# Makiato1999/HRI-EMO

Measured on AMD Instinct MI355X. Metric: utterances/sec fwd+bwd, d=768 T_a=400 T_t=128 N_e=6, higher is better.
Workload: dtype bf16; 1 GPU; FusionWithEmotionDecoder fwd+bwd (train mode, dropout 0.1), d=768 T_a=400 T_t=128 N_e=6 H=8, 2 fusion + 2 decoder layers, all-False masks (BASELINE cfg2); global_batch=64, batch_per_gpu=64, parallelism=dp1, grad_allreduce=none, launch=hipGraph replay, streams=2

## Files before the change

### hri-emo_amd/_lib.py

```python
import ctypes
import os

_HERE = os.path.dirname(os.path.abspath(__file__))
LIB_PATH = os.environ.get("HRIEMO_LIB") or os.path.join(_HERE, "libhriemo.so")

_C = {"p": ctypes.c_void_p, "i": ctypes.c_int, "l": ctypes.c_long, "f": ctypes.c_float,
      "Q": ctypes.c_ulonglong, "I": ctypes.c_uint}

_SIGS = {
    "hriemo_gemm_bf16": ("iiiiiplplplipipliplp", "i"),
    "hriemo_gemm_force_config": ("i", "i"),
    "hriemo_gemm_debug_flags": ("i", "i"),
    "hriemo_gemm_colsum_rows": ("iiiii", "i"),
    "hriemo_gemm_plan": ("iiiiiilppp", "i"),
    "hriemo_gemm_bf16_group_tn": ("piip", "i"),
    "hriemo_gemm_bf16_split": ("iiiiiplplplpliiplp", "i"),
    "hriemo_gemm_bf16_colsum": ("iiiiiplplplplpp", "i"),
    "hriemo_mx8_scale_ld": ("i", "l"),
    "hriemo_quant_mx8": ("pliiiplplp", "i"),
    "hriemo_gemm_mx8": ("iiiplplplplplipiplp", "i"),
    "hriemo_gemm_mx8_q": ("iiiplplplplplpiplplp", "i"),
    "hriemo_gemm_mx8_force_config": ("i", "i"),
    "hriemo_attn_fwd": ("plplplplppiiiiifQpIipp", "i"),
    "hriemo_attn_fwd_q": ("plplplplppiiiiifQpIipplplp", "i"),
    "hriemo_attn_bwd": ("plplplplplplplplpppiiiiifQpIipppp", "i"),
    "hriemo_attn_fwd_varlen": ("plplplplpppiiiiifQpIipp", "i"),
    "hriemo_attn_fwd_q_varlen": ("plplplplpppiiiiifQpIipplpllp", "i"),
    "hriemo_attn_bwd_varlen": ("plplplplplplplplppppiiiiifQpIipppp", "i"),
    "hriemo_attn_mask_bytes": ("iiii", "l"),
    "hriemo_attn_bwd_single_pass": ("iiii", "i"),
    "hriemo_attn_bwd_single_pass_q": ("iiiii", "i"),
    "hriemo_attn_bwd_kv_colsum_rows": ("iiiii", "i"),
    "hriemo_attn_bwd_colsum_rows": ("iiii", "i"),
    "hriemo_attn_bwd_dq_colsum_rows": ("iiiii", "i"),
    "hriemo_attn_plan": ("iiiiiipppppp", "i"),
    "hriemo_split_bf16x3": ("pliipiip", "i"),
    "hriemo_attn_fwd_f32": ("plplplplppiiiiifQpIip", "i"),
    "hriemo_attn_probs_f32": ("plplpppiiiiifQpIip", "i"),
# ... 122 lines not shown
```

### hri-emo_amd/_ops.py

```python
import itertools
import os as _os
import threading
from collections import namedtuple

import torch

from . import _lib

BF16 = torch.bfloat16
_EPS = 1e-5
_apply_tls = threading.local()


def _stream():
    return torch.cuda.current_stream().cuda_stream


def _p(t):
    return None if t is None else t.data_ptr()


def _require_fp32_master(p):
    if p.dtype != torch.float32:
        raise TypeError(f"hri_emo_amd: parameter of dtype {p.dtype}; keep the module's parameters in fp32 "
# ... 440 lines not shown

def fold_ffn_bias():
    return FOLD_FFN_BIAS


def linear_dx_masked_colsum(dy, w16, aux, bias_out, accumulate):
    M, N = dy.shape
    K = w16.shape[1]
    dx = torch.empty((M, K), dtype=BF16, device=dy.device)
    rows = _lib.lib().hriemo_gemm_colsum_rows(0, 1, M, K, N)
    part = torch.empty(rows * K, dtype=torch.float32, device=dy.device)
    _lib.call("hriemo_gemm_bf16_colsum", 0, 1, M, K, N, _p(dy), dy.stride(0), _p(w16), w16.stride(0), _p(dx), K, _p(aux), aux.stride(0),
              _p(part), _stream())
    if accumulate and DEFER_REDUCE and _in_backward():
        _deferred.add(part, K, rows, K, 1, [bias_out], True)
    else:
        red = _DeferredReduce()
        red.device = dy.device
        red.add(part, K, rows, K, 1, [bias_out], accumulate, schedule=False)
        red.flush()
    return dx


def linear_dw(dy, x, out, accumulate=False):
    M, N = dy.shape
    K = x.shape[1]
    if accumulate and M <= SMALL_DW_ROWS and _small_dw.enabled():
        _small_dw.add(dy, x, out)
        return
    gemm(1, 1, N, K, M, dy, dy.stride(0), x, x.stride(0), out, out.stride(0), c_f32=True, accumulate=accumulate)


def linear_dw_split(dy, x, out, out2, split, accumulate=False):
    M, N = dy.shape
    K = x.shape[1]
    ws = workspace(64 << 20, out.device)
    _lib.call("hriemo_gemm_bf16_split", 1, 1, N, K, M, _p(dy), dy.stride(0), _p(x), x.stride(0), _p(out), out.stride(0), _p(out2),
              out2.stride(0), split, int(accumulate), _p(ws), ws.numel() * 4, _stream())


GEMM_MODE = None


def set_gemm_mode(mode):
    global GEMM_MODE
    if mode not in ("bf16", "mx_fp8"):
        raise ValueError(f"gemm mode {mode!r}: expected 'bf16' or 'mx_fp8'")
    GEMM_MODE = mode


def gemm_mode():
    global GEMM_MODE
    if GEMM_MODE is None:
        import os
        GEMM_MODE = os.environ.get("HRIEMO_GEMM", "bf16")
        if GEMM_MODE not in ("bf16", "mx_fp8"):
            raise ValueError(f"HRIEMO_GEMM={GEMM_MODE!r}: expected 'bf16' or 'mx_fp8'")
    return GEMM_MODE


PRECISION = None
# ... 1001 lines not shown

def _attn_ln_fwd(ctx, head, q, k, v, x2, x32v, ar, H, hd, sh, w_in16, w_out16, drop, need_w, out_l, shape):
    p, seed, site, b_off = drop
    _, _, w_out, b_out, gamma, beta = ctx.params
    o, lse, *mbits = attn_fwd(q, k, v, ar.B, H, ar.Lq, ar.Lk, hd, ar.kpm, p, seed, site, b_off,
                              want_bits=attn_mask_bits(ar.B, H, ar.Lk, hd, ar.Lq), cu=ar.cu)
    g, y, y32, mean, rstd, mx = _proj_ln(o, sh, w_out, w_out16, b_out, x2, x32v, gamma, beta, p, seed, site + 1, b_off * ar.stride,
                                         ar.rows)
    probs = attn_probs(q, k, ar.B, H, ar.Lq, ar.Lk, hd, ar.kpm, lse, p, seed, site, b_off, ar.cu, out_l) if need_w else None
    ctx.save_for_backward(*head, o, lse, g, mean, rstd, w_in16, w_out16, gamma, mbits[0] if mbits else None)
    ctx.rows = ar
    ctx.mark_non_differentiable(*([probs] if probs is not None else []))
    return tag_mx(y.view(shape), mx), (y32.view(shape) if y32 is not None else None), probs


def _ln_bwd(params, dy, dy32, g, x2, x32v, gamma, mean, rstd, p, seed, site, row_off, rows, want_dx=True):
    dy2 = _contig_bf16(_sum_grads(dy, dy32)).view(x2.shape)
    sink = GradSink(params)
    return (sink,) + add_ln_bwd(dy2, g, x2, gamma, mean, rstd, p, seed, site, row_off, want_dx=want_dx,
                                outs=(sink.buf(params[-2]), sink.buf(params[-1]), sink.buf(params[-3])),
                                accumulate=sink.fused, x32=x32v, rows=rows)


def _attn_ln_bwd(ctx, params, dy, dy32, x2, x32v, tail, want_dx=True):
    o, lse, g, mean, rstd, w_in16, w_out16, gamma, mbits = tail
    p, seed, site, b_off = ctx.cfg[-4:]
    sink, ds, dg, dgamma, dbeta, db_out = _ln_bwd(params, dy, dy32, g, x2, x32v, gamma, mean, rstd, p, seed, site + 1,
                                                  b_off * ctx.rows.stride, ctx.rows.rows, want_dx)
    dw_out = sink.buf(params[-4])
    linear_dw(dg, o, dw_out, sink.fused)
    return sink, ds, linear_dx(dg, w_out16), dw_out, db_out, dgamma, dbeta


class SelfAttnLN(_GradModeAware, torch.autograd.Function):

    @staticmethod
    def forward(ctx, x, x32, w_in, b_in, w_out, b_out, gamma, beta, sh, H, seq, p, seed, site, b_off, need_w):
        seq.holds(x)
        if precision() == "fp32":
            return _fp32().self_attn_ln(ctx, x, x32, w_in, b_in, w_out, b_out, gamma, beta, sh, H, seq, need_w, p, seed, site, b_off)
        _require_fp32_masters(w_in, b_in, w_out, b_out, gamma, beta)
        ctx.set_materialize_grads(False)
        _require_gpu(x)
        B, L, d = x.shape
        hd = _heads(d, H)
        M = B * L
        ar = attn_rows(seq, seq, need_w)
        x2 = _contig_bf16(x).view(M, d)
        x32 = _c32(x32)
        x32v = x32.view(M, d) if x32 is not None else None
        w_in16, w_out16 = sh.get(w_in), sh.get(w_out)
        ctx.cfg = (B, L, d, H, hd, p, seed, site, b_off)
        ctx.params = (w_in, b_in, w_out, b_out, gamma, beta)
        qkv = proj_fwd(Operand(x2, mx_of(x)), sh, w_in, w_in16, b_in)
        return _attn_ln_fwd(ctx, (x2, x32v, qkv), qkv[:, :d], qkv[:, d:2 * d], qkv[:, 2 * d:], x2, x32v, ar, H, hd, sh, w_in16,
                            w_out16, (p, seed, site, b_off), need_w, (seq.L, seq.L), (B, L, d))

    @staticmethod
    def backward(ctx, dy, dy32, _dprobs):
        if getattr(ctx, "fp32", False):
            return _fp32().self_attn_ln_bwd(ctx, dy, dy32)
        x2, x32v, qkv, o, lse, _, _, _, w_in16, _, _, mbits = saved = ctx.saved_tensors
        B, L, d, H, hd, p, seed, site, b_off = ctx.cfg
        ar = ctx.rows
        M = B * L
        p_w_in, p_b_in = ctx.params[:2]
        want_dx = ctx.needs_input_grad[0] or ctx.needs_input_grad[1] or FORCE_INPUT_GRAD
        sink, ds, do, dw_out, db_out, dgamma, dbeta = _attn_ln_bwd(ctx, ctx.params, dy, dy32, x2, x32v, saved[-9:], want_dx)
        acc = sink.fused
        dqkv = torch.empty((M, 3 * d), dtype=BF16, device=x2.device)
        db_in = sink.buf(p_b_in)
        folded = attn_bwd(qkv[:, :d], qkv[:, d:2 * d], qkv[:, 2 * d:], o, do, dqkv[:, :d], dqkv[:, d:2 * d], dqkv[:, 2 * d:],
                          lse, ar.B, H, ar.Lq, ar.Lk, hd, ar.kpm, p, seed, site, b_off, bias_grad=(db_in[:d], db_in[d:], acc), mask_bits=mbits,
                          cu=ar.cu)
        dw_in = sink.buf(p_w_in)
        linear_dw(dqkv, x2, dw_in, acc)
        if not folded:
            colsum(dqkv, db_in, acc)
        dx = linear_dx(dqkv, w_in16, epi=3, aux=ds).view(B, L, d) if want_dx else None
        sink.done()
        if site in FLUSH_SITES:
            _small_dw.flush()
        r = sink.ret
        return (dx, None, r(dw_in), r(db_in), r(dw_out), r(db_out), r(dgamma), r(dbeta)) + (None,) * 8


class CrossAttnLN(_GradModeAware, torch.autograd.Function):

    @staticmethod
    def forward(ctx, xq, xq32, xkv, w_in, b_in, w_out, b_out, gamma, beta, sh, H, seq_q, seq_k, p, seed, site, b_off, need_w,
                kv_pre=None, join_q=None, q_pre=None, slots=None):
        if (q_pre is None) != (slots is None) or (q_pre is not None and kv_pre is None):
            raise ValueError("CrossAttnLN: q_pre and slots come together, and only with kv_pre (both projections made by SharedProjFn)")
        seq_q.holds(xq)
        seq_k.holds(xkv)
        if precision() == "fp32":
            return _fp32().cross_attn_ln(ctx, xq, xq32, xkv, w_in, b_in, w_out, b_out, gamma, beta, sh, H, seq_q, seq_k, need_w, p, seed,
                                         site, b_off)
        _require_fp32_masters(w_in, b_in, w_out, b_out, gamma, beta)
# ... 9 lines not shown
        ctx.cfg = (B, Lq, Lk, d, H, hd, p, seed, site, b_off)
        ctx.params = (w_in, b_in, w_out, b_out, gamma, beta)
        ctx.own_q, ctx.own_kv, ctx.slots, ctx.join_q = q_pre is None, kv_pre is None, slots, join_q
        w_out16 = sh.get(w_out)
        w_in16 = sh.get(w_in) if (ctx.own_q or ctx.own_kv) else None
        q = q_pre if q_pre is not None else proj_fwd(Operand(xq2, mx_of(xq)), sh, w_in, w_in16, b_in, rows=(0, d))
        if kv_pre is not None:
            xkv2, kv = None, kv_pre
        else:
            xkv2 = _contig_bf16(xkv).view(B * Lk, d)
            kv = proj_fwd(Operand(xkv2, mx_of(xkv)), sh, w_in, w_in16, b_in, rows=(d, 3 * d))
        return _attn_ln_fwd(ctx, (xq2, x32v, xkv2, q, kv), q, kv[:, :d], kv[:, d:], xq2, x32v, ar, H, hd, sh, w_in16,
                            w_out16, (p, seed, site, b_off), need_w, (seq_q.L, seq_k.L), (B, Lq, d))

    @staticmethod
    def backward(ctx, dy, dy32, _dprobs):
        if getattr(ctx, "fp32", False):
            return _fp32().cross_attn_ln_bwd(ctx, dy, dy32)
        xq2, x32v, xkv2, q, kv, o, lse, _, _, _, w_in16, _, _, mbits = saved = ctx.saved_tensors
        B, Lq, Lk, d, H, hd, p, seed, site, b_off = ctx.cfg
        ar = ctx.rows
        own_q, own_kv = ctx.own_q, ctx.own_kv
        p_w_in, p_b_in = ctx.params[:2]
        sink, ds, do, dw_out, db_out, dgamma, dbeta = _attn_ln_bwd(ctx, ctx.params if own_q else ctx.params[1:], dy, dy32, xq2, x32v, saved[-9:])
        acc = sink.fused
        if own_q:
            dq = torch.empty((B * Lq, d), dtype=BF16, device=xq2.device)
            dkv = (torch.zeros if ar.kv_surplus else torch.empty)((B * Lk, 2 * d), dtype=BF16, device=xq2.device)
        else:
            dq, dkv = ctx.slots[0].buf(), ctx.slots[1].buf()
        db_in = sink.buf(p_b_in)
        folded = attn_bwd(q, kv[:, :d], kv[:, d:], o, do, dq, dkv[:, :d], dkv[:, d:], lse, ar.B, H, ar.Lq, ar.Lk, hd, ar.kpm, p, seed,
                          site, b_off, bias_grad=(db_in[:d], db_in[d:], acc), mask_bits=mbits, cu=ar.cu)
        dw_in = None
        if own_q:
            dw_in = sink.buf(p_w_in)
            linear_dw(dq, xq2, dw_in[:d], acc)
        if not folded:
            colsum(dq, db_in[:d], acc)
            colsum(dkv, db_in[d:], acc)
        dxq = linear_dx(dq, w_in16[:d], epi=3, aux=ds) if own_q else ds
        if ctx.join_q is not None:
            last, dep = ctx.join_q.arrive()
            if dep is not None:
                dxq = dxq + dep.view(B * Lq, d)
            if not last:
                ctx.join_q.deposit(dxq)
                dxq = None
        dxq = dxq.view(B, Lq, d) if dxq is not None else None
        dxkv = None
        if own_kv:
            linear_dw(dkv, xkv2, dw_in[d:], acc)
            dxkv = linear_dx(dkv, w_in16[d:]).view(B, Lk, d)
        elif own_q and not acc:
            dw_in[d:].zero_()
        sink.done(skip=() if own_kv else (p_w_in,))
        r = sink.ret
        return (dxq, None, dxkv, r(dw_in), r(db_in), r(dw_out), r(db_out), r(dgamma), r(dbeta)) + (None,) * 9 + \
            (None if own_kv else dkv, None, None if own_q else dq, None)


class GradJoin:

    def __init__(self, n=2):
        self.n, self.seen, self.dep, self.ev = n, 0, None, None

    def arrive(self):
        if self.seen == 0:
            torch.autograd.Variable._execution_engine.queue_callback(self._check)
        self.seen += 1
        last = self.seen == self.n
        dep, ev = self.dep, self.ev
        self.dep = self.ev = None
        if last:
            self.seen = 0
# ... 204 lines not shown
                DROP_LOG.append(("rows", seed, site + 2, M, h.shape[1], float(p_mid), b_off * L))
            _lib.call("hriemo_dropout_bf16", _p(h), _p(hd_), M, h.shape[1], float(p_mid), seed, _p(seed_word(h.device)),
                      site + 2, b_off * L, _stream())
        g, y, y32, mean, rstd, mx = _proj_ln(hd_, sh, w2, w2_16, b2, x2, x32v, gamma, beta, p, seed, site + 1, b_off * seq.L, seq.idx)
        ctx.save_for_backward(x2, x32v, h, hd_, g, mean, rstd, w1_16, w2_16, gamma)
        ctx.cfg = (B, L, d, p, p_mid, seed, site, b_off)
        ctx.seq = seq
        ctx.params = (w1, b1, w2, b2, gamma, beta)
        return tag_mx(y.view(B, L, d), mx), (y32.view(B, L, d) if y32 is not None else None)

    @staticmethod
    def backward(ctx, dy, dy32):
        if getattr(ctx, "fp32", False):
            return _fp32().ffn_ln_bwd(ctx, dy, dy32)
        x2, x32v, h, hd_, g, mean, rstd, w1_16, w2_16, gamma = ctx.saved_tensors
        B, L, d, p, p_mid, seed, site, b_off = ctx.cfg
        M, F = h.shape
        dev = x2.device
        p_w1, p_b1, p_w2 = ctx.params[:3]
        sink, ds, dg, dgamma, dbeta, db2 = _ln_bwd(ctx.params, dy, dy32, g, x2, x32v, gamma, mean, rstd, p, seed, site + 1,
                                                   b_off * ctx.seq.L, ctx.seq.idx)
        acc = sink.fused
        dw2 = sink.buf(p_w2)
        linear_dw(dg, hd_, dw2, acc)
        db1 = sink.buf(p_b1)
        fold = p_mid == 0 and fold_ffn_bias()
        if fold:
            da = linear_dx_masked_colsum(dg, w2_16, h, db1, acc)
        else:
            da = linear_dx(dg, w2_16, epi=2, aux=h)
        if p_mid > 0:
            _lib.call("hriemo_dropout_bf16", _p(da), _p(da), M, F, float(p_mid), seed, _p(seed_word(dev)), site + 2, b_off * L,
                      _stream())
        dw1 = sink.buf(p_w1)
        linear_dw(da, x2, dw1, acc)
        if not fold:
            colsum(da, db1, acc)
        dx = linear_dx(da, w1_16, epi=3, aux=ds)
        sink.done()
        r = sink.ret
        return (dx.view(B, L, d), None, r(dw1), r(db1), r(dw2), r(db2), r(dgamma), r(dbeta)) + (None,) * 7


class BetaGateFn(_GradModeAware, torch.autograd.Function):

    @staticmethod
    def forward(ctx, h_a, h_a32, h_t, h_t32, ga, ba, gt, bt, w1, b1, w2, b2, sh, sa, st, sf):
        if not (sa.packed == st.packed == sf.packed):
            raise ValueError("BetaGate: the three layouts must be all padded or all packed")
        B, La, Lt, d = sa.Breal, sa.L, st.L, h_a.shape[-1]
        Ra, Rt = h_a.shape[0] * h_a.shape[1], h_t.shape[0] * h_t.shape[1]
        if Ra != sa.N or Rt != st.N:
            raise ValueError(f"BetaGate: packed rows {Ra} / {Rt} do not match the plan ({sa.N} / {st.N})")
        L = La if La == Lt else Lt
        if La < L:
            raise RuntimeError(f"BetaGate: audio length {La} < text length {Lt}; the reference cannot fuse this either")
        if precision() == "fp32":
            return _fp32().beta_gate(ctx, h_a, h_a32, h_t, h_t32, ga, ba, gt, bt, w1, b1, w2, b2, sh, sa, st, sf)
# ... 373 lines not shown
```

### hri-emo_amd/csrc/gemm.hip

```cpp
#include "gemm_common.h"
#include <string.h>
#include <stdlib.h>

template <int TA, int TB, int OUTF32, int BM, int BN, int WM, int WN, int NS, int BK>
__device__ __forceinline__ void gemm_body(const GemmArgs& p) {
  constexpr int NWAVE = WM * WN;
  constexpr bool K32 = (BK == 32), STAG = K32 && (WM * WN == 8);
  constexpr int A_BYTES = BM * BK * 2, B_BYTES = BN * BK * 2, STAGE = A_BYTES + B_BYTES;
  constexpr int A_PW = A_BYTES / 1024 / NWAVE, B_PW = B_BYTES / 1024 / NWAVE, LPT = A_PW + B_PW;
  constexpr int MT = BM / WM / 16, NTL = BN / WN / 16;
  static_assert(A_PW * NWAVE * 1024 == A_BYTES && B_PW * NWAVE * 1024 == B_BYTES, "tile must split evenly over waves");
  static_assert(NS >= 2 && NS <= 8 && (NS - 1) * LPT < 64, "ring depth / vmcnt range");
  static_assert(!STAG || NS == 4, "staggered schedule: 4 ring slots");
  static_assert(!K32 || NS >= 3, "32-deep stages need a ring of 3");
  extern __shared__ __attribute__((aligned(16))) char smem[];
  const int tid = threadIdx.x, lane = tid & 63;
  const int wave = __builtin_amdgcn_readfirstlane(tid >> 6);
  const int wm = wave / WN, wn = wave % WN;
  char* scratch = smem + NS * STAGE + wave * 2048;

  const int G = gridDim.x, nxcd = min(8, G), q = G / nxcd, r = G - q * nxcd;
  const int xcd = blockIdx.x % nxcd, lb = blockIdx.x / nxcd, nx = q + (xcd < r ? 1 : 0);
  const int before = xcd * q + min(xcd, r);
  const int tiles = p.tiles_m * p.tiles_n;
// ... 311 lines not shown
    if (!has_next) break;
    if (!OUTF32) {
      const int rows_valid = p.M - (T.m0 + wm * MT * 16), cols_valid = p.N - (T.n0 + wn * 64);
      relax_first = (p.flags & 1) && rows_valid >= MT * 16 && cols_valid >= 64 && p.cs == nullptr;
    }
    T = decode(nwg);
    wg = nwg;
    if (dyn) {
      if (tid == 0) qslot[0] = drawn;
      __builtin_amdgcn_s_waitcnt(0xC07F);
      parked = true;
    } else {
      nwg = wg + nx;
    }
  }
  leave();
}

template <int TA, int TB, int OUTF32, int BM, int BN, int WM, int WN, int NS, int BK>
__global__ __launch_bounds__(WM * WN * 64, (WM * WN == 4 ? 2 : 1)) void gemm_kernel(const GemmArgs p) {
  gemm_body<TA, TB, OUTF32, BM, BN, WM, WN, NS, BK>(p);
}

template <int TA, int TB, int OUTF32>
__global__ __launch_bounds__(768) void gemm_ws_kernel(const GemmArgs p) {
  constexpr int BM = 256, BN = 128, BK = 64, NS = 3, WN = 2, NCW = 8, NLW = 4, MT = 4, NTL = 4;
  constexpr int A_BYTES = BM * BK * 2, B_BYTES = BN * BK * 2, STAGE = A_BYTES + B_BYTES;
  constexpr int A_PL = A_BYTES / 1024 / NLW, B_PL = B_BYTES / 1024 / NLW, LPL = A_PL + B_PL;
  extern __shared__ __attribute__((aligned(16))) char smem[];
  const int tid = threadIdx.x, lane = tid & 63;
  const int wave = __builtin_amdgcn_readfirstlane(tid >> 6);
  const int G = gridDim.x, nxcd = min(8, G), q = G / nxcd, r = G - q * nxcd;
  const int xcd = blockIdx.x % nxcd, lb = blockIdx.x / nxcd, nx = q + (xcd < r ? 1 : 0);
  const int before = xcd * q + min(xcd, r);
  const int tiles = p.tiles_m * p.tiles_n;
  const long total = (long)tiles * p.splitk;
  const int end = (int)(total * (before + nx) / G), beg = (int)(total * before / G);
  const bool dyn = p.sched != nullptr;
  unsigned* const qctr = p.sched + xcd;
  int* const qslot = (int*)(smem + NS * STAGE);
  const int wg0 = beg + lb, wg1 = wg0 + nx;
  auto leave = [&]() {
    if (dyn && tid == 0) {
      const unsigned done = atomicAdd(p.sched + 8, 1u);
      if (done == gridDim.x - 1) {
#pragma unroll
        for (int k = 0; k < 9; ++k) __hip_atomic_store(p.sched + k, 0u, __ATOMIC_RELAXED, __HIP_MEMORY_SCOPE_AGENT);
      }
    }
  };
  if (wg0 >= end) { leave(); return; }
  auto decode = [&](int w) {
    TileInfo t;
    t.slice = w / tiles;
    const int rr = w - t.slice * tiles;
    const int tm = rr / p.tiles_n, tn = rr - tm * p.tiles_n;
    t.m0 = tm * BM; t.n0 = tn * BN;
    const int kbeg = t.slice * p.k_per_split;
    t.kext = min(p.K, kbeg + p.k_per_split) - kbeg;
    t.nk = (t.kext + BK - 1) / BK;
    t.abase = TA == 0 ? p.A + (long)t.m0 * p.lda + kbeg : p.A + (long)kbeg * p.lda + t.m0;
    t.bbase = TB == 0 ? p.B + (long)t.n0 * p.ldb + kbeg : p.B + (long)kbeg * p.ldb + t.n0;
    t.a_valid = p.M - t.m0; t.b_valid = p.N - t.n0;
    return t;
  };
  if (wave >= NCW) {
    __builtin_amdgcn_s_setprio(3);
    const int lw = wave - NCW;
    const long astep = TA == 0 ? BK : BK * p.lda, bstep = TB == 0 ? BK : BK * p.ldb;
    const LaneOff aoff = operand_lane<TA, BM, BK>(p.lda, lane), boff = operand_lane<TB, BN, BK>(p.ldb, lane);
    int ik = 0, islot = 0;
    int known_next = dyn ? end : wg1;
    bool more = true, crossed = false;
    TileInfo IT = decode(wg0);
    auto issue_next = [&]() -> bool {
      if (crossed) {
        crossed = false;
        if (known_next < end) IT = decode(known_next); else more = false;
      }
      if (!more) return false;
      char* sa = smem + islot * STAGE;
      const int krem = IT.kext - ik * BK;
      stage_operand<TA, BM, A_PL, BK>(sa, IT.abase + ik * astep, aoff, p.lda, IT.a_valid, krem, lw, lane);
      stage_operand<TB, BN, B_PL, BK>(sa + A_BYTES, IT.bbase + ik * bstep, boff, p.ldb, IT.b_valid, krem, lw, lane);
      islot = (islot + 1 == NS) ? 0 : islot + 1;
      if (++ik == IT.nk) { ik = 0; crossed = true; }
      return true;
    };
    int pending = 0;
    if (issue_next()) ++pending;
    if (issue_next()) ++pending;
    for (int w = wg0; w < end;) {
      const int nk = decode(w).nk;
      for (int it = 0; it < nk; ++it) {
        if (pending >= 2) wait_vmcnt<LPL>(); else wait_vmcnt<0>();
        __builtin_amdgcn_s_barrier();
        if (dyn && it == nk - 2) {
          const int v = *(LDS_PTR(const int))qslot;
          __builtin_amdgcn_s_waitcnt(0xC07F);
          known_next = __builtin_amdgcn_readfirstlane(v);
        }
        --pending;
        if (issue_next()) ++pending;
      }
      w = known_next;
      if (!dyn) known_next = w + nx;
    }
// ... 4 lines not shown
  f32x4 acc[MT][NTL];
  auto load_frags = [&](const char* sa, int ks, bf16x8 (&af)[MT], bf16x8 (&bfr)[NTL]) {
    const char* sb = sa + A_BYTES;
#pragma unroll
    for (int mi = 0; mi < MT; ++mi)
      af[mi] = TA == 0 ? lds_row_frag<BK>(sa, wm * MT * 16 + mi * 16, ks, lane) : lds_tr_frag<BM * 2>(sa, wm * MT * 16 + mi * 16, ks, lane);
#pragma unroll
    for (int ni = 0; ni < NTL; ++ni)
      bfr[ni] = TB == 0 ? lds_row_frag<BK>(sb, wn * NTL * 16 + ni * 16, ks, lane) : lds_tr_frag<BN * 2>(sb, wn * NTL * 16 + ni * 16, ks, lane);
  };
  auto mma = [&](const bf16x8 (&af)[MT], const bf16x8 (&bfr)[NTL]) {
#pragma unroll
    for (int mi = 0; mi < MT; ++mi)
#pragma unroll
      for (int ni = 0; ni < NTL; ++ni)
        acc[mi][ni] = __builtin_amdgcn_mfma_f32_16x16x32_bf16(bfr[ni], af[mi], acc[mi][ni], 0, 0, 0);
  };
  constexpr int RD = (TA == 0 ? 1 : 2) * MT + (TB == 0 ? 1 : 2) * NTL;
  int cur = 0;
  const bool drawer = dyn && wave == 0;
  int drawn = end, nextv = dyn ? end : wg1;
  if (drawer && lane == 0) drawn = (int)atomicAdd(qctr, 1u);
  for (int w = wg0; w < end;) {
    const TileInfo T = decode(w);
#pragma unroll
    for (int a = 0; a < MT; ++a)
#pragma unroll
      for (int b = 0; b < NTL; ++b) acc[a][b] = (f32x4){0.f, 0.f, 0.f, 0.f};
    bf16x8 afA[MT], bfA[NTL], afB[MT], bfB[NTL];
    auto interleave = [&]() {
#pragma unroll
      for (int gq = 0; gq < 4; ++gq) {
        __builtin_amdgcn_sched_group_barrier(0x008, MT * NTL / 4, 0);
        __builtin_amdgcn_sched_group_barrier(0x100, (RD + 3) / 4, 0);
      }
    };
    {
      if (drawer && T.nk == 2 && lane == 0) qslot[0] = beg + nx + drawn;
      __builtin_amdgcn_s_waitcnt(0xC07F);
      __builtin_amdgcn_s_barrier();
      __builtin_amdgcn_sched_barrier(0);
      if (dyn && T.nk == 2) nextv = *(LDS_PTR(const int))qslot;
      const char* sa = smem + cur * STAGE;
      load_frags(sa, 0, afA, bfA);
      load_frags(sa, 1, afB, bfB);
      mma(afA, bfA);
      __builtin_amdgcn_sched_group_barrier(0x100, RD, 0);
// ... 2 lines not shown
      cur = (cur + 1 == NS) ? 0 : cur + 1;
    }
    for (int it = 1; it < T.nk; ++it) {
      if (drawer && it == T.nk - 2 && lane == 0) qslot[0] = beg + nx + drawn;
      __builtin_amdgcn_s_waitcnt(0xC07F);
      __builtin_amdgcn_s_barrier();
      __builtin_amdgcn_sched_barrier(0);
      if (dyn && it == T.nk - 2) nextv = *(LDS_PTR(const int))qslot;
      const char* sa = smem + cur * STAGE;
      load_frags(sa, 0, afA, bfA);
      mma(afB, bfB);
      interleave();
      __builtin_amdgcn_sched_barrier(0);
      load_frags(sa, 1, afB, bfB);
      mma(afA, bfA);
      interleave();
      __builtin_amdgcn_sched_barrier(0);
      cur = (cur + 1 == NS) ? 0 : cur + 1;
    }
    __builtin_amdgcn_s_waitcnt(0xC07F);
    mma(afB, bfB);
    if (drawer && lane == 0) drawn = (int)atomicAdd(qctr, 1u);
    if (OUTF32) {
      store_tile<1, 0, MT, NTL>(acc, p, T, scratch, wm, wn, lane);
    } else {
      switch (p.epi) {
        case 1: store_tile<0, 1, MT, NTL>(acc, p, T, scratch, wm, wn, lane); break;
        case 2: store_tile<0, 2, MT, NTL>(acc, p, T, scratch, wm, wn, lane); break;
        case 3: store_tile<0, 3, MT, NTL>(acc, p, T, scratch, wm, wn, lane); break;
        default: store_tile<0, 0, MT, NTL>(acc, p, T, scratch, wm, wn, lane); break;
      }
    }
    w = __builtin_amdgcn_readfirstlane(nextv);
    nextv = dyn ? end : w + nx;
  }
  leave();
}

struct GemmGroup { GemmArgs p[16]; };
template <int TA, int TB, int OUTF32, int BM, int BN, int WM, int WN, int NS, int BK>
__global__ __launch_bounds__(WM * WN * 64, (WM * WN == 4 ? 2 : 1)) void gemm_group_kernel(const GemmGroup grp) {
  gemm_body<TA, TB, OUTF32, BM, BN, WM, WN, NS, BK>(grp.p[blockIdx.y]);
}

__global__ __launch_bounds__(256) void splitk_reduce_kernel(const float* __restrict__ ws, float* __restrict__ C, long ldc, int M, int N,
                                                            int splitk, int accumulate, float* __restrict__ C2, long ldc2, int split_m) {
  const long nv = (long)M * N / 4, slab = (long)M * N;
  for (long v = (long)blockIdx.x * blockDim.x + threadIdx.x; v < nv; v += (long)gridDim.x * blockDim.x) {
    const long e = v * 4;
    const int m = (int)(e / N), n = (int)(e - (long)m * N);
    const float* src = ws + e;
    float* dst = m < split_m ? C + (long)m * ldc + n : C2 + (long)(m - split_m) * ldc2 + n;
    f32x4 c = {0.f, 0.f, 0.f, 0.f};
    if (accumulate) c = *(const f32x4*)dst;
    f32x4 s = *(const f32x4*)src;
    int k = 1;
    for (; k + 4 <= splitk; k += 4) {
      const f32x4 a0 = *(const f32x4*)(src + (k + 0) * slab), a1 = *(const f32x4*)(src + (k + 1) * slab);
      const f32x4 a2 = *(const f32x4*)(src + (k + 2) * slab), a3 = *(const f32x4*)(src + (k + 3) * slab);
      s += a0; s += a1; s += a2; s += a3;
    }
    for (; k < splitk; ++k) s += *(const f32x4*)(src + k * slab);
    if (accumulate) s += c;
    *(f32x4*)dst = s;
  }
}

struct TileCfg { int bm, bn, threads, lds, ns, bk; };
static const TileCfg kCfg[] = {
    {128, 128, 256, 2 * 32768, 2, 64},
    {256, 128, 512, 3 * 49152, 3, 64},
    {256, 256, 512, 2 * 65536, 2, 64},
    {64, 128, 256, 4 * 24576, 4, 64},
    {256, 256, 512, 4 * 32768, 4, 32},
    {320, 128, 512, 2 * 57344, 2, 64},
    {64, 128, 256, 6 * 24576, 6, 64},
    {32, 128, 256, 7 * 20480, 7, 64},
    {32, 64, 128, 6 * 12288, 6, 64},
    {256, 128, 768, 3 * 49152, 3, 64},
};
static const int kNumCfg = sizeof(kCfg) / sizeof(kCfg[0]);
int hriemo_num_cus() {
  static int n = 0;
  if (n == 0) {
    int dev = 0;
    hipGetDevice(&dev);
    if (hipDeviceGetAttribute(&n, hipDeviceAttributeMultiprocessorCount, dev) != hipSuccess || n <= 0) n = 256;
  }
// ... 243 lines not shown
      a.M = (int)r[0]; a.N = (int)r[1]; a.K = (int)r[2];
      a.A = (const bf16_t*)r[3]; a.lda = (long)r[4]; a.B = (const bf16_t*)r[5]; a.ldb = (long)r[6]; a.C = (void*)r[7]; a.ldc = (long)r[8];
      HRIEMO_CHECK(a.M > 0 && a.N > 0 && a.K > 0 && a.M % 8 == 0 && a.N % 8 == 0, "gemm_group: job %d: bad shape %dx%dx%d", j0 + j, a.M, a.N, a.K);
      HRIEMO_CHECK(a.lda % 8 == 0 && a.ldb % 8 == 0 && a.ldc % 4 == 0 && ((uintptr_t)a.A % 16) == 0 && ((uintptr_t)a.B % 16) == 0 &&
                       ((uintptr_t)a.C % 16) == 0 && a.lda < (1L << 21) && a.ldb < (1L << 21), "gemm_group: job %d: alignment", j0 + j);
      HRIEMO_CHECK(a.K > (kCfg[0].ns - 2) * kCfg[0].bk, "gemm_group: job %d: reduction too short for the operand ring", j0 + j);
      a.tiles_m = (a.M + BM - 1) / BM; a.tiles_n = (a.N + BN - 1) / BN;
      a.splitk = 1; a.k_per_split = (a.K + 63) / 64 * 64;
      a.accumulate = accumulate; a.sched = nullptr;
      const int tiles = a.tiles_m * a.tiles_n;
      if (tiles > gx) gx = tiles;
      flops += 2.0 * a.M * a.N * a.K;
    }
    for (int j = nj; j < 16; ++j) { g.p[j] = g.p[0]; g.p[j].tiles_m = 0; g.p[j].tiles_n = 0; }
    const int cap = 2 * hriemo_num_cus();
    if (gx > cap) gx = cap;
    hriemo_prof_begin(HP_GEMM_TN, st);
    hipLaunchKernelGGL(kern, dim3(gx, nj), dim3(256), lds, st, g);
    HRIEMO_LAUNCH_CHECK("gemm_group_kernel");
    hriemo_prof_end(HP_GEMM_TN, st, flops);
  }
  return 0;
}
extern "C" int hriemo_gemm_bf16_colsum(int ta, int tb, int M, int N, int K, const void* A, long lda, const void* B, long ldb,
                                       void* C, long ldc, const void* aux, long ldaux, float* colsum_partials, hipStream_t st) {
  HRIEMO_CHECK(colsum_partials != nullptr, "gemm_colsum: partials buffer missing");
  return gemm_impl(ta, tb, M, N, K, A, lda, B, ldb, C, ldc, 0, nullptr, 2, aux, ldaux, 0, nullptr, 0, colsum_partials, st);
}
```

### include/hriemo.h

```cpp
#ifndef HRIEMO_H_
#define HRIEMO_H_

#ifdef __cplusplus
extern "C" {
#endif

typedef struct ihipStream_t* hriemo_stream_t;

const char* hriemo_last_error(void);
int hriemo_abi_version(void);

int hriemo_gemm_bf16(int ta, int tb, int M, int N, int K, const void* A, long lda, const void* B, long ldb,
                     void* C, long ldc, int c_is_f32, const float* bias, int epilogue, const void* aux,
                     long ldaux, int accumulate, float* workspace, long workspace_bytes, hriemo_stream_t stream);

int hriemo_gemm_bf16_group_tn(const void* jobs_host, int njobs, int accumulate, hriemo_stream_t stream);
int hriemo_gemm_bf16_split(int ta, int tb, int M, int N, int K, const void* A, long lda, const void* B, long ldb, void* C, long ldc,
                           void* C2, long ldc2, int split_m, int accumulate, float* workspace, long workspace_bytes,
                           hriemo_stream_t stream);
int hriemo_gemm_colsum_rows(int ta, int tb, int M, int N, int K);
int hriemo_gemm_bf16_colsum(int ta, int tb, int M, int N, int K, const void* A, long lda, const void* B, long ldb, void* C, long ldc,
                            const void* aux, long ldaux, float* colsum_partials, hriemo_stream_t stream);
int hriemo_gemm_force_config(int cfg);
int hriemo_gemm_debug_flags(int flags);
int hriemo_gemm_plan(int ta, int tb, int M, int N, int K, int c_is_f32, long workspace_bytes, int* cfg, int* splitk,
                     int* k_per_split);

long hriemo_mx8_scale_ld(int rows);
int hriemo_quant_mx8(const void* X, long ldx, int src_is_f32, int M, int K, void* Xq, long ldq, void* S, long lds,
                     hriemo_stream_t stream);
int hriemo_gemm_mx8(int M, int N, int K, const void* Aq, long lda, const void* SA, long ldsa, const void* Bq, long ldb,
                    const void* SB, long ldsb, void* C, long ldc, int c_is_f32, const float* bias, int epilogue,
                    const void* aux, long ldaux, hriemo_stream_t stream);
int hriemo_gemm_mx8_q(int M, int N, int K, const void* Aq, long lda, const void* SA, long ldsa, const void* Bq, long ldb,
                      const void* SB, long ldsb, void* C, long ldc, const float* bias, int epilogue, void* CQ, long ldcq,
                      void* SC, long ldsc, hriemo_stream_t stream);
int hriemo_gemm_mx8_force_config(int cfg);

int hriemo_attn_fwd(const void* Q, long ldq, const void* K, long ldk, const void* V, long ldv, void* O, long ldo,
// ... 266 lines not shown
```

Measured before the change: 8850 utterances/s.

## Group attention weight-gradient GEMMs into one persistent split-K launch

Adds a grouped variant of the warp-specialized persistent GEMM kernel that schedules tiles from up to four weight-gradient problems in a single launch. A planner picks per-problem split-K so the combined units fill the CUs, and a grouped reduce kernel then sums the split-K partials. Self-attention in/out projection dW and cross-attention q/kv/out dW are batched this way during backward, which cuts launch count and the tail underutilization of small dW GEMMs. The cost is extra split-K workspace traffic, a reduce pass, and per-tile problem decoding inside the kernel.

```diff
diff --git a/hri-emo_amd/_lib.py b/hri-emo_amd/_lib.py
--- a/hri-emo_amd/_lib.py
+++ b/hri-emo_amd/_lib.py
@@ -14,6 +14,8 @@
     "hriemo_gemm_colsum_rows": ("iiiii", "i"),
     "hriemo_gemm_plan": ("iiiiiilppp", "i"),
     "hriemo_gemm_bf16_group_tn": ("piip", "i"),
+    "hriemo_gemm_bf16_group_tn_ws": ("piiplp", "i"),
+    "hriemo_gemm_group_plan": ("pilpppp", "i"),
     "hriemo_gemm_bf16_split": ("iiiiiplplplpliiplp", "i"),
     "hriemo_gemm_bf16_colsum": ("iiiiiplplplplpp", "i"),
     "hriemo_mx8_scale_ld": ("i", "l"),
diff --git a/hri-emo_amd/_ops.py b/hri-emo_amd/_ops.py
--- a/hri-emo_amd/_ops.py
+++ b/hri-emo_amd/_ops.py
@@ -486,11 +486,14 @@
     return dx
 
 
-def linear_dw(dy, x, out, accumulate=False):
+def linear_dw(dy, x, out, accumulate=False, group=None):
     M, N = dy.shape
     K = x.shape[1]
     if accumulate and M <= SMALL_DW_ROWS and _small_dw.enabled():
         _small_dw.add(dy, x, out)
+        return
+    if group is not None:
+        group.add(dy, x, out)
         return
     gemm(1, 1, N, K, M, dy, dy.stride(0), x, x.stride(0), out, out.stride(0), c_f32=True, accumulate=accumulate)
 
@@ -501,6 +504,36 @@
     ws = workspace(64 << 20, out.device)
     _lib.call("hriemo_gemm_bf16_split", 1, 1, N, K, M, _p(dy), dy.stride(0), _p(x), x.stride(0), _p(out), out.stride(0), _p(out2),
               out2.stride(0), split, int(accumulate), _p(ws), ws.numel() * 4, _stream())
+
+
+GROUP_DW = True
+GROUP_DW_SITES = "self_attn+cross_attn"
+
+
+class _DwGroup:
+
+    def __init__(self):
+        self.jobs = []
+
+    def add(self, dy, x, out):
+        self.jobs.append((dy, x, out))
+
+    def issue(self, accumulate):
+        jobs, self.jobs = self.jobs, []
+        if len(jobs) == 1:
+            linear_dw(*jobs[0], accumulate)
+        elif jobs:
+            ws = workspace(64 << 20, jobs[0][2].device)
+            table = [(dy.shape[1], x.shape[1], dy.shape[0], dy.data_ptr(), dy.stride(0), x.data_ptr(), x.stride(0), out.data_ptr(),
+                      out.stride(0), 0, 0, 0) for dy, x, out in jobs]
+            host = torch.tensor(table, dtype=torch.int64)
+            _lib.call("hriemo_gemm_bf16_group_tn_ws", host.data_ptr(), len(table), int(accumulate), _p(ws), ws.numel() * 4, _stream())
+
+
+def dw_group(site):
+    if GROUP_DW and site in GROUP_DW_SITES.split("+") and _in_backward() and not grad_hooks_active() and precision() != "fp32":
+        return _DwGroup()
+    return None
 
 
 GEMM_MODE = None
@@ -1548,13 +1581,13 @@
                                 accumulate=sink.fused, x32=x32v, rows=rows)
 
 
-def _attn_ln_bwd(ctx, params, dy, dy32, x2, x32v, tail, want_dx=True):
+def _attn_ln_bwd(ctx, params, dy, dy32, x2, x32v, tail, want_dx=True, group=None):
     o, lse, g, mean, rstd, w_in16, w_out16, gamma, mbits = tail
     p, seed, site, b_off = ctx.cfg[-4:]
     sink, ds, dg, dgamma, dbeta, db_out = _ln_bwd(params, dy, dy32, g, x2, x32v, gamma, mean, rstd, p, seed, site + 1,
                                                   b_off * ctx.rows.stride, ctx.rows.rows, want_dx)
     dw_out = sink.buf(params[-4])
-    linear_dw(dg, o, dw_out, sink.fused)
+    linear_dw(dg, o, dw_out, sink.fused, group)
     return sink, ds, linear_dx(dg, w_out16), dw_out, db_out, dgamma, dbeta
 
 
@@ -1592,7 +1625,8 @@
         M = B * L
         p_w_in, p_b_in = ctx.params[:2]
         want_dx = ctx.needs_input_grad[0] or ctx.needs_input_grad[1] or FORCE_INPUT_GRAD
-        sink, ds, do, dw_out, db_out, dgamma, dbeta = _attn_ln_bwd(ctx, ctx.params, dy, dy32, x2, x32v, saved[-9:], want_dx)
+        grp = dw_group("self_attn")
+        sink, ds, do, dw_out, db_out, dgamma, dbeta = _attn_ln_bwd(ctx, ctx.params, dy, dy32, x2, x32v, saved[-9:], want_dx, grp)
         acc = sink.fused
         dqkv = torch.empty((M, 3 * d), dtype=BF16, device=x2.device)
         db_in = sink.buf(p_b_in)
@@ -1600,7 +1634,9 @@
                           lse, ar.B, H, ar.Lq, ar.Lk, hd, ar.kpm, p, seed, site, b_off, bias_grad=(db_in[:d], db_in[d:], acc), mask_bits=mbits,
                           cu=ar.cu)
         dw_in = sink.buf(p_w_in)
-        linear_dw(dqkv, x2, dw_in, acc)
+        linear_dw(dqkv, x2, dw_in, acc, grp)
+        if grp is not None:
+            grp.issue(acc)
         if not folded:
             colsum(dqkv, db_in, acc)
         dx = linear_dx(dqkv, w_in16, epi=3, aux=ds).view(B, L, d) if want_dx else None
@@ -1656,7 +1692,9 @@
         ar = ctx.rows
         own_q, own_kv = ctx.own_q, ctx.own_kv
         p_w_in, p_b_in = ctx.params[:2]
-        sink, ds, do, dw_out, db_out, dgamma, dbeta = _attn_ln_bwd(ctx, ctx.params if own_q else ctx.params[1:], dy, dy32, xq2, x32v, saved[-9:])
+        grp = dw_group("cross_attn") if own_q else None
+        sink, ds, do, dw_out, db_out, dgamma, dbeta = _attn_ln_bwd(ctx, ctx.params if own_q else ctx.params[1:], dy, dy32, xq2, x32v, saved[-9:],
+                                                                   group=grp)
         acc = sink.fused
         if own_q:
             dq = torch.empty((B * Lq, d), dtype=BF16, device=xq2.device)
@@ -1669,7 +1707,11 @@
         dw_in = None
         if own_q:
             dw_in = sink.buf(p_w_in)
-            linear_dw(dq, xq2, dw_in[:d], acc)
+            linear_dw(dq, xq2, dw_in[:d], acc, grp)
+            if grp is not None:
+                if own_kv:
+                    linear_dw(dkv, xkv2, dw_in[d:], acc, grp)
+                grp.issue(acc)
         if not folded:
             colsum(dq, db_in[:d], acc)
             colsum(dkv, db_in[d:], acc)
@@ -1684,7 +1726,8 @@
         dxq = dxq.view(B, Lq, d) if dxq is not None else None
         dxkv = None
         if own_kv:
-            linear_dw(dkv, xkv2, dw_in[d:], acc)
+            if grp is None:
+                linear_dw(dkv, xkv2, dw_in[d:], acc)
             dxkv = linear_dx(dkv, w_in16[d:]).view(B, Lk, d)
         elif own_q and not acc:
             dw_in[d:].zero_()
@@ -1935,7 +1978,8 @@
                                                    b_off * ctx.seq.L, ctx.seq.idx)
         acc = sink.fused
         dw2 = sink.buf(p_w2)
-        linear_dw(dg, hd_, dw2, acc)
+        grp = dw_group("ffn")
+        linear_dw(dg, hd_, dw2, acc, grp)
         db1 = sink.buf(p_b1)
         fold = p_mid == 0 and fold_ffn_bias()
         if fold:
@@ -1946,7 +1990,9 @@
             _lib.call("hriemo_dropout_bf16", _p(da), _p(da), M, F, float(p_mid), seed, _p(seed_word(dev)), site + 2, b_off * L,
                       _stream())
         dw1 = sink.buf(p_w1)
-        linear_dw(da, x2, dw1, acc)
+        linear_dw(da, x2, dw1, acc, grp)
+        if grp is not None:
+            grp.issue(acc)
         if not fold:
             colsum(da, db1, acc)
         dx = linear_dx(da, w1_16, epi=3, aux=ds)
diff --git a/hri-emo_amd/csrc/gemm.hip b/hri-emo_amd/csrc/gemm.hip
--- a/hri-emo_amd/csrc/gemm.hip
+++ b/hri-emo_amd/csrc/gemm.hip
@@ -357,8 +357,23 @@
   gemm_body<TA, TB, OUTF32, BM, BN, WM, WN, NS, BK>(p);
 }
 
-template <int TA, int TB, int OUTF32>
-__global__ __launch_bounds__(768) void gemm_ws_kernel(const GemmArgs p) {
+struct GemmWsGroup {
+  GemmArgs p[4];
+  int ustart[4];
+  int total;
+  unsigned* sched;
+};
+struct TileInfoG : TileInfo { int pi; };
+__device__ __forceinline__ const GemmArgs& ws_first(const GemmArgs& a) { return a; }
+__device__ __forceinline__ const GemmArgs& ws_first(const GemmWsGroup& a) { return a.p[0]; }
+template <int TA, int TB, int OUTF32, typename ArgT = GemmArgs>
+__global__ __launch_bounds__(768) void gemm_ws_kernel(const ArgT g) {
+  constexpr bool GRP = std::is_same<ArgT, GemmWsGroup>::value;
+  typedef typename std::conditional<GRP, TileInfoG, TileInfo>::type TileT;
+  const GemmArgs& p = ws_first(g);
+  auto prob = [&](int pi) -> const GemmArgs& {
+    if constexpr (GRP) return g.p[pi]; else return p;
+  };
   constexpr int BM = 256, BN = 128, BK = 64, NS = 3, WN = 2, NCW = 8, NLW = 4, MT = 4, NTL = 4;
   constexpr int A_BYTES = BM * BK * 2, B_BYTES = BN * BK * 2, STAGE = A_BYTES + B_BYTES;
   constexpr int A_PL = A_BYTES / 1024 / NLW, B_PL = B_BYTES / 1024 / NLW, LPL = A_PL + B_PL;
@@ -369,24 +384,24 @@
   const int xcd = blockIdx.x % nxcd, lb = blockIdx.x / nxcd, nx = q + (xcd < r ? 1 : 0);
   const int before = xcd * q + min(xcd, r);
   const int tiles = p.tiles_m * p.tiles_n;
-  const long total = (long)tiles * p.splitk;
+  long total = (long)tiles * p.splitk;
+  if constexpr (GRP) total = g.total;
   const int end = (int)(total * (before + nx) / G), beg = (int)(total * before / G);
-  const bool dyn = p.sched != nullptr;
-  unsigned* const qctr = p.sched + xcd;
+  const bool dyn = g.sched != nullptr;
+  unsigned* const qctr = g.sched + xcd;
   int* const qslot = (int*)(smem + NS * STAGE);
   const int wg0 = beg + lb, wg1 = wg0 + nx;
   auto leave = [&]() {
     if (dyn && tid == 0) {
-      const unsigned done = atomicAdd(p.sched + 8, 1u);
+      const unsigned done = atomicAdd(g.sched + 8, 1u);
       if (done == gridDim.x - 1) {
 #pragma unroll
-        for (int k = 0; k < 9; ++k) __hip_atomic_store(p.sched + k, 0u, __ATOMIC_RELAXED, __HIP_MEMORY_SCOPE_AGENT);
+        for (int k = 0; k < 9; ++k) __hip_atomic_store(g.sched + k, 0u, __ATOMIC_RELAXED, __HIP_MEMORY_SCOPE_AGENT);
       }
     }
   };
   if (wg0 >= end) { leave(); return; }
-  auto decode = [&](int w) {
-    TileInfo t;
+  auto decode_in = [&](const GemmArgs& p, int tiles, int w, TileT& t) {
     t.slice = w / tiles;
     const int rr = w - t.slice * tiles;
     const int tm = rr / p.tiles_n, tn = rr - tm * p.tiles_n;
@@ -397,6 +412,16 @@
     t.abase = TA == 0 ? p.A + (long)t.m0 * p.lda + kbeg : p.A + (long)kbeg * p.lda + t.m0;
     t.bbase = TB == 0 ? p.B + (long)t.n0 * p.ldb + kbeg : p.B + (long)kbeg * p.ldb + t.n0;
     t.a_valid = p.M - t.m0; t.b_valid = p.N - t.n0;
+  };
+  auto decode = [&](int w) {
+    TileT t;
+    if constexpr (GRP) {
+      const int pi = (w >= g.ustart[1]) + (w >= g.ustart[2]) + (w >= g.ustart[3]);
+      t.pi = pi;
+      decode_in(g.p[pi], g.p[pi].tiles_m * g.p[pi].tiles_n, w - g.ustart[pi], t);
+    } else {
+      decode_in(p, tiles, w, t);
+    }
     return t;
   };
   if (wave >= NCW) {
@@ -404,20 +429,34 @@
     const int lw = wave - NCW;
     const long astep = TA == 0 ? BK : BK * p.lda, bstep = TB == 0 ? BK : BK * p.ldb;
     const LaneOff aoff = operand_lane<TA, BM, BK>(p.lda, lane), boff = operand_lane<TB, BN, BK>(p.ldb, lane);
+    struct { long lda, ldb, astep, bstep; LaneOff aoff, boff; } gq = {p.lda, p.ldb, astep, bstep, aoff, boff};
+    auto enter = [&](const TileT& t) {
+      if constexpr (GRP) {
+        gq.lda = g.p[t.pi].lda; gq.ldb = g.p[t.pi].ldb;
+        gq.astep = TA == 0 ? BK : BK * gq.lda; gq.bstep = TB == 0 ? BK : BK * gq.ldb;
+        gq.aoff = operand_lane<TA, BM, BK>(gq.lda, lane); gq.boff = operand_lane<TB, BN, BK>(gq.ldb, lane);
+      }
+    };
     int ik = 0, islot = 0;
     int known_next = dyn ? end : wg1;
     bool more = true, crossed = false;
-    TileInfo IT = decode(wg0);
+    TileT IT = decode(wg0);
+    enter(IT);
     auto issue_next = [&]() -> bool {
       if (crossed) {
         crossed = false;
-        if (known_next < end) IT = decode(known_next); else more = false;
+        if (known_next < end) { IT = decode(known_next); enter(IT); } else more = false;
       }
       if (!more) return false;
       char* sa = smem + islot * STAGE;
       const int krem = IT.kext - ik * BK;
-      stage_operand<TA, BM, A_PL, BK>(sa, IT.abase + ik * astep, aoff, p.lda, IT.a_valid, krem, lw, lane);
-      stage_operand<TB, BN, B_PL, BK>(sa + A_BYTES, IT.bbase + ik * bstep, boff, p.ldb, IT.b_valid, krem, lw, lane);
+      if constexpr (GRP) {
+        stage_operand<TA, BM, A_PL, BK>(sa, IT.abase + ik * gq.astep, gq.aoff, gq.lda, IT.a_valid, krem, lw, lane);
+        stage_operand<TB, BN, B_PL, BK>(sa + A_BYTES, IT.bbase + ik * gq.bstep, gq.boff, gq.ldb, IT.b_valid, krem, lw, lane);
+      } else {
+        stage_operand<TA, BM, A_PL, BK>(sa, IT.abase + ik * astep, aoff, p.lda, IT.a_valid, krem, lw, lane);
+        stage_operand<TB, BN, B_PL, BK>(sa + A_BYTES, IT.bbase + ik * bstep, boff, p.ldb, IT.b_valid, krem, lw, lane);
+      }
       islot = (islot + 1 == NS) ? 0 : islot + 1;
       if (++ik == IT.nk) { ik = 0; crossed = true; }
       return true;
@@ -468,7 +507,10 @@
   int drawn = end, nextv = dyn ? end : wg1;
   if (drawer && lane == 0) drawn = (int)atomicAdd(qctr, 1u);
   for (int w = wg0; w < end;) {
-    const TileInfo T = decode(w);
+    const TileT T = decode(w);
+    int tpi = 0;
+    if constexpr (GRP) tpi = T.pi;
+    const GemmArgs& pt = prob(tpi);
 #pragma unroll
     for (int a = 0; a < MT; ++a)
 #pragma unroll
@@ -517,13 +559,13 @@
     mma(afB, bfB);
     if (drawer && lane == 0) drawn = (int)atomicAdd(qctr, 1u);
     if (OUTF32) {
-      store_tile<1, 0, MT, NTL>(acc, p, T, scratch, wm, wn, lane);
+      store_tile<1, 0, MT, NTL>(acc, pt, T, scratch, wm, wn, lane);
     } else {
-      switch (p.epi) {
-        case 1: store_tile<0, 1, MT, NTL>(acc, p, T, scratch, wm, wn, lane); break;
-        case 2: store_tile<0, 2, MT, NTL>(acc, p, T, scratch, wm, wn, lane); break;
-        case 3: store_tile<0, 3, MT, NTL>(acc, p, T, scratch, wm, wn, lane); break;
-        default: store_tile<0, 0, MT, NTL>(acc, p, T, scratch, wm, wn, lane); break;
+      switch (pt.epi) {
+        case 1: store_tile<0, 1, MT, NTL>(acc, pt, T, scratch, wm, wn, lane); break;
+        case 2: store_tile<0, 2, MT, NTL>(acc, pt, T, scratch, wm, wn, lane); break;
+        case 3: store_tile<0, 3, MT, NTL>(acc, pt, T, scratch, wm, wn, lane); break;
+        default: store_tile<0, 0, MT, NTL>(acc, pt, T, scratch, wm, wn, lane); break;
       }
     }
     w = __builtin_amdgcn_readfirstlane(nextv);
@@ -538,10 +580,10 @@
   gemm_body<TA, TB, OUTF32, BM, BN, WM, WN, NS, BK>(grp.p[blockIdx.y]);
 }
 
-__global__ __launch_bounds__(256) void splitk_reduce_kernel(const float* __restrict__ ws, float* __restrict__ C, long ldc, int M, int N,
-                                                            int splitk, int accumulate, float* __restrict__ C2, long ldc2, int split_m) {
+__device__ __forceinline__ void splitk_reduce_rows(const float* __restrict__ ws, float* __restrict__ C, long ldc, int M, int N, int splitk,
+                                                   int accumulate, float* __restrict__ C2, long ldc2, int split_m, long blk, long nblk) {
   const long nv = (long)M * N / 4, slab = (long)M * N;
-  for (long v = (long)blockIdx.x * blockDim.x + threadIdx.x; v < nv; v += (long)gridDim.x * blockDim.x) {
+  for (long v = blk * blockDim.x + threadIdx.x; v < nv; v += nblk * blockDim.x) {
     const long e = v * 4;
     const int m = (int)(e / N), n = (int)(e - (long)m * N);
     const float* src = ws + e;
@@ -559,6 +601,19 @@
     if (accumulate) s += c;
     *(f32x4*)dst = s;
   }
+}
+__global__ __launch_bounds__(256) void splitk_reduce_kernel(const float* __restrict__ ws, float* __restrict__ C, long ldc, int M, int N,
+                                                            int splitk, int accumulate, float* __restrict__ C2, long ldc2, int split_m) {
+  splitk_reduce_rows(ws, C, ldc, M, N, splitk, accumulate, C2, ldc2, split_m, blockIdx.x, gridDim.x);
+}
+struct ReduceJob { const float* ws; float* C; float* C2; long ldc, ldc2; int M, N, splitk, split_m, accumulate; };
+struct ReduceGroup { ReduceJob j[4]; int bstart[5]; };
+__global__ __launch_bounds__(256) void splitk_reduce_group_kernel(const ReduceGroup rg) {
+  const int b = blockIdx.x;
+  const int ji = (b >= rg.bstart[1]) + (b >= rg.bstart[2]) + (b >= rg.bstart[3]);
+  const ReduceJob& J = rg.j[ji];
+  splitk_reduce_rows(J.ws, J.C, J.ldc, J.M, J.N, J.splitk, J.accumulate, J.C2, J.ldc2, J.split_m, b - rg.bstart[ji],
+                     rg.bstart[ji + 1] - rg.bstart[ji]);
 }
 
 struct TileCfg { int bm, bn, threads, lds, ns, bk; };
@@ -848,6 +903,165 @@
   }
   return 0;
 }
+struct GroupProb { int M, N, K, needs_split; };
+struct GroupPlan { int in_group[4], splitk[4], k_per_split[4], units; };
+static GroupPlan plan_group(int n, const GroupProb* pr, long workspace_bytes) {
+  GroupPlan best = {};
+  const long slots = hriemo_num_cus();
+  int ks[4], smax[4];
+  long tiles[4];
+  int ng = 0;
+  for (int i = 0; i < n; ++i) {
+    tiles[i] = (long)((pr[i].M + 255) / 256) * ((pr[i].N + 127) / 128);
+    ks[i] = (pr[i].K + 63) / 64;
+    smax[i] = ks[i] / 16;
+    const bool ok = smax[i] >= (pr[i].needs_split ? 2 : 1) && pr[i].M % 8 == 0 && pr[i].N % 8 == 0;
+    best.in_group[i] = ok;
+    best.splitk[i] = 1;
+    best.k_per_split[i] = ks[i] * 64;
+    ng += ok;
+  }
+  auto none = [&]() { for (int i = 0; i < n; ++i) best.in_group[i] = 0; best.units = 0; return best; };
+  if (ng < 2) return none();
+  double best_cost = -1.0;
+  int best_slices = 0;
+  GroupPlan cand = best;
+  for (int ci = 0; ci < n; ++ci) {
+    if (!best.in_group[ci]) continue;
+    for (int cs = 1; cs <= smax[ci]; ++cs) {
+      const int L = (ks[ci] + cs - 1) / cs;
+      long units = 0, slab_bytes = 0;
+      int longest = 0, slices = 0;
+      bool valid = true;
+      for (int i = 0; i < n && valid; ++i) {
+        if (!best.in_group[i]) continue;
+        int s = (ks[i] + L - 1) / L;
+        if (s > smax[i]) s = smax[i];
+        if (pr[i].needs_split && s < 2) s = 2;
+        int kper = 0;
+        for (;; --s) {
+          kper = ((pr[i].K + s - 1) / s + 63) / 64 * 64;
+          const int sl = (pr[i].K + kper - 1) / kper;
+          const int last = pr[i].K - (sl - 1) * kper;
+          if (sl == s && (last + 63) / 64 >= 16) break;
+          if (sl < s) { s = sl + 1; continue; }
+          if (s == 1) break;
+        }
+        if (pr[i].needs_split && s < 2) { valid = false; break; }
+        cand.splitk[i] = s; cand.k_per_split[i] = kper;
+        units += tiles[i] * s;
+        slices += s;
+        if (kper / 64 > longest) longest = kper / 64;
+        if (s > 1) slab_bytes += (long)s * pr[i].M * pr[i].N * 4;
+      }
+      if (!valid || units > 2 * slots || slab_bytes > workspace_bytes) continue;
+      const double cost = (double)((units + slots - 1) / slots) * longest + (double)slab_bytes / (2 << 20);
+      if (best_cost < 0.0 || cost < best_cost || (cost == best_cost && slices < best_slices)) {
+        best_cost = cost; best_slices = slices;
+        for (int i = 0; i < n; ++i) { best.splitk[i] = cand.splitk[i]; best.k_per_split[i] = cand.k_per_split[i]; }
+        best.units = (int)units;
+      }
+    }
+  }
+  if (best_cost < 0.0) return none();
+  return best;
+}
+static void group_probs(const long long* h, int njobs, GroupProb* pr) {
+  for (int j = 0; j < njobs; ++j) pr[j] = {(int)h[j * 12 + 0], (int)h[j * 12 + 1], (int)h[j * 12 + 2], h[j * 12 + 9] != 0};
+}
+extern "C" int hriemo_gemm_group_plan(const void* jobs_host, int njobs, long workspace_bytes, int* in_group, int* splitk, int* k_per_split,
+                                      int* units) {
+  HRIEMO_CHECK(jobs_host != nullptr && njobs > 0 && njobs <= 4, "gemm_group_plan: 1..4 jobs");
+  HRIEMO_CHECK(in_group != nullptr && splitk != nullptr && k_per_split != nullptr && units != nullptr, "gemm_group_plan: bad arguments");
+  GroupProb pr[4];
+  group_probs((const long long*)jobs_host, njobs, pr);
+  for (int j = 0; j < njobs; ++j) HRIEMO_CHECK(pr[j].M > 0 && pr[j].N > 0 && pr[j].K > 0, "gemm_group_plan: job %d: empty problem", j);
+  const GroupPlan pl = plan_group(njobs, pr, workspace_bytes > 0 ? workspace_bytes : 0);
+  for (int j = 0; j < njobs; ++j) { in_group[j] = pl.in_group[j]; splitk[j] = pl.splitk[j]; k_per_split[j] = pl.k_per_split[j]; }
+  *units = pl.units;
+  return 0;
+}
+extern "C" int hriemo_gemm_bf16_group_tn_ws(const void* jobs_host, int njobs, int accumulate, float* workspace, long workspace_bytes,
+                                            hipStream_t st) {
+  HRIEMO_CHECK(jobs_host != nullptr && njobs > 0 && njobs <= 4, "gemm_group_ws: 1..4 jobs");
+  const long long* h = (const long long*)jobs_host;
+  GroupProb pr[4];
+  group_probs(h, njobs, pr);
+  for (int j = 0; j < njobs; ++j) {
+    const long long* r = h + j * 12;
+    HRIEMO_CHECK(pr[j].M > 0 && pr[j].N > 0 && pr[j].K > 0 && pr[j].M % 8 == 0 && pr[j].N % 8 == 0, "gemm_group_ws: job %d: bad shape %dx%dx%d", j,
+                 pr[j].M, pr[j].N, pr[j].K);
+    HRIEMO_CHECK(r[4] % 8 == 0 && r[6] % 8 == 0 && r[8] % 4 == 0 && ((uintptr_t)r[3] % 16) == 0 && ((uintptr_t)r[5] % 16) == 0 &&
+                     ((uintptr_t)r[7] % 16) == 0 && r[4] < (1L << 21) && r[6] < (1L << 21), "gemm_group_ws: job %d: alignment", j);
+    HRIEMO_CHECK(r[9] == 0 || (r[11] > 0 && r[11] < r[0] && r[10] % 4 == 0 && ((uintptr_t)r[9] % 16) == 0),
+                 "gemm_group_ws: job %d: a split output needs 0 < split_m < M and a 16-byte aligned second matrix", j);
+  }
+  const GroupPlan pl = plan_group(njobs, pr, workspace != nullptr ? workspace_bytes : 0);
+  if (pl.units > 0) {
+    GemmWsGroup g = {};
+    ReduceGroup rg = {};
+    int order[4], ng = 0, nr = 0;
+    for (int j = 0; j < njobs; ++j) if (pl.in_group[j]) order[ng++] = j;
+    for (int a = 1; a < ng; ++a)
+      for (int b = a; b > 0 && pl.k_per_split[order[b]] > pl.k_per_split[order[b - 1]]; --b) { const int t = order[b]; order[b] = order[b - 1]; order[b - 1] = t; }
+    long ws_off = 0;
+    int unit0 = 0, blk0 = 0;
+    double flops = 0.0;
+    for (int i = 0; i < ng; ++i) {
+      const int j = order[i];
+      const long long* r = h + j * 12;
+      GemmArgs& a = g.p[i];
+      a.M = pr[j].M; a.N = pr[j].N; a.K = pr[j].K;
+      a.A = (const bf16_t*)r[3]; a.lda = (long)r[4]; a.B = (const bf16_t*)r[5]; a.ldb = (long)r[6]; a.C = (void*)r[7]; a.ldc = (long)r[8];
+      a.tiles_m = (a.M + 255) / 256; a.tiles_n = (a.N + 127) / 128;
+      a.splitk = pl.splitk[j]; a.k_per_split = pl.k_per_split[j];
+      a.accumulate = accumulate; a.flags = g_gemm_flags;
+      g.ustart[i] = unit0;
+      unit0 += a.tiles_m * a.tiles_n * a.splitk;
+      if (a.splitk > 1) {
+        a.ws = workspace + ws_off;
+        ws_off += (long)a.splitk * a.M * a.N;
+        ReduceJob& q = rg.j[nr];
+        q.ws = a.ws; q.C = (float*)a.C; q.ldc = a.ldc; q.C2 = (float*)r[9]; q.ldc2 = (long)r[10];
+        q.M = a.M; q.N = a.N; q.splitk = a.splitk; q.split_m = r[9] != 0 ? (int)r[11] : a.M; q.accumulate = accumulate;
+        const long nv = (long)a.M * a.N / 4;
+        long nb = (nv + 255) / 256;
+        if (nb > 16L * hriemo_num_cus()) nb = 16L * hriemo_num_cus();
+        rg.bstart[nr++] = blk0;
+        blk0 += (int)nb;
+      }
+      flops += 2.0 * a.M * a.N * a.K;
+    }
+    HRIEMO_CHECK(unit0 == pl.units && ws_off * 4 <= workspace_bytes, "gemm_group_ws: plan and launch disagree");
+    for (int i = ng; i < 4; ++i) { g.p[i] = g.p[0]; g.ustart[i] = unit0; }
+    for (int i = nr; i < 5; ++i) rg.bstart[i] = blk0;
+    g.total = unit0;
+    const long slots = hriemo_num_cus();
+    g.sched = (unit0 > slots && !(g_gemm_flags & 8)) ? hriemo_gemm_sched_slot(st) : nullptr;
+    const int wlds = kCfg[9].lds + 8 * 2048;
+    static bool attr_set = false;
+    if (!attr_set) {
+      hipFuncSetAttribute((const void*)gemm_ws_kernel<1, 1, 1, GemmWsGroup>, hipFuncAttributeMaxDynamicSharedMemorySize, wlds);
+      attr_set = true;
+    }
+    hriemo_prof_begin(HP_GEMM_TN, st);
+    hipLaunchKernelGGL((gemm_ws_kernel<1, 1, 1, GemmWsGroup>), dim3((int)(unit0 < slots ? unit0 : slots)), dim3(768), wlds, st, g);
+    HRIEMO_LAUNCH_CHECK("gemm_ws_kernel (grouped)");
+    if (nr > 0) {
+      hipLaunchKernelGGL(splitk_reduce_group_kernel, dim3(blk0), dim3(256), 0, st, rg);
+      HRIEMO_LAUNCH_CHECK("splitk_reduce_group_kernel");
+    }
+    hriemo_prof_end(HP_GEMM_TN, st, flops);
+  }
+  for (int j = 0; j < njobs; ++j) {
+    if (pl.units > 0 && pl.in_group[j]) continue;
+    const long long* r = h + j * 12;
+    const int rc = gemm_impl(1, 1, pr[j].M, pr[j].N, pr[j].K, (const void*)r[3], (long)r[4], (const void*)r[5], (long)r[6], (void*)r[7], (long)r[8], 1,
+                             nullptr, 0, nullptr, 0, accumulate, workspace, workspace_bytes, nullptr, st, (void*)r[9], (long)r[10], (int)r[11]);
+    if (rc != 0) return rc;
+  }
+  return 0;
+}
 extern "C" int hriemo_gemm_bf16_colsum(int ta, int tb, int M, int N, int K, const void* A, long lda, const void* B, long ldb,
                                        void* C, long ldc, const void* aux, long ldaux, float* colsum_partials, hipStream_t st) {
   HRIEMO_CHECK(colsum_partials != nullptr, "gemm_colsum: partials buffer missing");
diff --git a/include/hriemo.h b/include/hriemo.h
--- a/include/hriemo.h
+++ b/include/hriemo.h
@@ -15,6 +15,10 @@
                      long ldaux, int accumulate, float* workspace, long workspace_bytes, hriemo_stream_t stream);
 
 int hriemo_gemm_bf16_group_tn(const void* jobs_host, int njobs, int accumulate, hriemo_stream_t stream);
+int hriemo_gemm_bf16_group_tn_ws(const void* jobs_host, int njobs, int accumulate, float* workspace, long workspace_bytes,
+                                 hriemo_stream_t stream);
+int hriemo_gemm_group_plan(const void* jobs_host, int njobs, long workspace_bytes, int* in_group, int* splitk, int* k_per_split,
+                           int* units);
 int hriemo_gemm_bf16_split(int ta, int tb, int M, int N, int K, const void* A, long lda, const void* B, long ldb, void* C, long ldc,
                            void* C2, long ldc2, int split_m, int accumulate, float* workspace, long workspace_bytes,
                            hriemo_stream_t stream);
```

Measured after the change: 8876 utterances/s (median of 4 runs). No clear change (+0.3%).
